# BBillot/SynthSR

Measured on AMD Instinct MI355X. Metric: training volumes/sec (160^3 fp32, 5-level U-Net), higher is better.
Workload: dtype f32; 1 GPU; configs[1]: brain_generator 160^3 batch=1 (training() defaults) + 5-level 3-D U-Net (24..384 features, Cin=2) fwd/bwd + Adam, fp32, random-init; global_batch=1, parallelism=dp1, conv_arithmetic=split

## Files before the change

### synthsr_amd/csrc/conv_split.hip

```cpp
#include "common.h"
#include <algorithm>
#include <type_traits>
#include <utility>

#ifdef SYN_SPLIT_TIMING
static __device__ long long* g_tm = nullptr;
extern "C" int synthsr_split_timing_buffer(long long* p) {
  return hipMemcpyToSymbol(HIP_SYMBOL(g_tm), &p, sizeof(p)) == hipSuccess ? 0 : 1;
}
#define TM(i) do { if (g_tm && (blockIdx.x == 0 || blockIdx.x == 300) && blockIdx.y == 0 && tid == 0 && tix < 120) g_tm[((blockIdx.x ? 1 : 0) * 120 + tix) * 8 + (i)] = clock64(); } while (0)
#define T2(k) do { if (g_tm && threadIdx.x == 0 && ((blockIdx.x == 7 && blockIdx.y == 0) || (blockIdx.x == 20 && blockIdx.y == 1)) && n2 < 400) { g_tm[(blockIdx.y * 400 + n2) * 2] = (k); g_tm[(blockIdx.y * 400 + n2) * 2 + 1] = clock64(); ++n2; } } while (0)
#else
#define TM(i)
#define T2(k)
#endif
#ifdef SYN_SPLIT_TIMING
#define T3(i) do { if (g_tm && lane == 0 && blockIdx.x == 7 && blockIdx.y == 0 && n3 < 48) g_tm[1600 + ((tid >> 6) * 48 + n3) * 2 + (i)] = clock64(); } while (0)
#else
#define T3(i)
#endif


namespace {

// ... 836 lines not shown
    int j = tid + NTHR * i;
    if (j >= NP) j -= NTHR;
    const int v = j >> 1, h = j & 1;
    const int hz = v / (HY * HX), r = v - hz * (HY * HX), hy = r / HX, hx = r - hy * HX;
    prel[i] = ((hz * D1 + hy) * D2 + hx) * Cin * 4 + h * 16;
    plds[i] = v * 16 + h * 8;
    pmask[i] = (1u << hz) | (1u << (6 + hy)) | (1u << (12 + hx));
  }
  const __amdgpu_buffer_rsrc_t rin =
      __builtin_amdgcn_make_buffer_rsrc(const_cast<float*>(a.in), 0, (int)((int64_t)D0 * D1 * D2 * Cin * 4), 0x00020000);
  f32x4 hst[NL], hnx[NL];
  auto halo_issue = [&](int t, int cc) {
    const bool none = t >= walk.end;
    int z0, y0, x0;
    tile_decode(none ? walk.pos : t, tiles0, a.tiles1, a.tiles2, z0, y0, x0);
    uint32_t bad = none ? 0xFFFFFFFFu : 0x80000000u;
    bad |= syn_oob_bits(z0 - 1, HZ, D0) | (syn_oob_bits(y0 - 1, HY, D1) << 6) | (syn_oob_bits(x0 - 1, HX, D2) << 12);
    const int base = ((((z0 - 1) * D1 + (y0 - 1)) * D2 + (x0 - 1)) * Cin + cc * 8) * 4;
#pragma unroll
    for (int i = 0; i < NL; ++i) {
      const uint32_t vo = (pmask[i] & bad) ? OOB : (uint32_t)(prel[i] + base);
      hnx[i] = __builtin_bit_cast(f32x4, __builtin_amdgcn_raw_buffer_load_b128(rin, (int)vo, 0, 0));
    }
  };
  typedef unsigned int u32x2 __attribute__((ext_vector_type(2)));
  uint32_t cp[6];
  auto conv_a = [&](int i) { syn_split3(hst[i][0], hst[i][1], cp[0], cp[1], cp[2]); };
  auto conv_b = [&](int i) { syn_split3(hst[i][2], hst[i][3], cp[3], cp[4], cp[5]); };
  auto conv_c = [&](int i, unsigned char* dst) {
    *reinterpret_cast<u32x2*>(dst + plds[i]) = (u32x2){cp[0], cp[3]};
    *reinterpret_cast<u32x2*>(dst + PLANE + plds[i]) = (u32x2){cp[1], cp[4]};
    *reinterpret_cast<u32x2*>(dst + 2 * PLANE + plds[i]) = (u32x2){cp[2], cp[5]};
  };

  const int piece_stride = nchunks * ncc * NSTEP * MT * 64;
  const __amdgpu_buffer_rsrc_t rw = __builtin_amdgcn_make_buffer_rsrc(
      const_cast<u32x4*>(a.wp), 0, (int)((int64_t)3 * piece_stride * 16), 0x00020000);
  int wsrc[C::NWL];
#pragma unroll
  for (int k = 0; k < C::NWL; ++k) {
    int j = tid + NTHR * k;
    if (j >= C::NWP) j = tid;
    const int q = j / (NSTEP * MT * 64), r = j - q * (NSTEP * MT * 64);
    wsrc[k] = (q * piece_stride + chunk * ncc * NSTEP * MT * 64 + r) * 16;
  }
  u32x4 wst[C::NWL];
  auto w_issue = [&](int cc) {
#pragma unroll
    for (int k = 0; k < C::NWL; ++k) wst[k] = __builtin_amdgcn_raw_buffer_load_b128(rw, wsrc[k] + cc * (NSTEP * MT * 64 * 16), 0, 0);
  };
  auto w_store = [&](unsigned char* dst) {
#pragma unroll
    for (int k = 0; k < C::NWL; ++k) {
      const int j = (tid + NTHR * k) >= C::NWP ? tid : tid + NTHR * k;
      *reinterpret_cast<u32x4*>(dst + j * 16) = wst[k];
    }
  };

  float s1[ST ? MT : 1][4], s2[ST ? MT : 1][4];
#pragma unroll
  for (int mt = 0; mt < (ST ? MT : 1); ++mt)
#pragma unroll
    for (int i = 0; i < 4; ++i) s1[mt][i] = s2[mt][i] = 0.f;

  const int64_t out_bytes = (int64_t)D0 * D1 * D2 * Cout * 4;
  const __amdgpu_buffer_rsrc_t rout = __builtin_amdgcn_make_buffer_rsrc(a.out, 0, (int)out_bytes, 0x00020000);
  const __amdgpu_buffer_rsrc_t radd = __builtin_amdgcn_make_buffer_rsrc(
      const_cast<float*>(a.addend ? a.addend : a.out), 0, (int)out_bytes, 0x00020000);
  const uint32_t ystep = (uint32_t)(D2 * Cout * 4);
  if (tid < MT * 16) {
    const int co = chunk * MT * 16 + tid;
    lbias[tid] = (a.bias && co < Cout) ? a.bias[co] : 0.f;
  }

  f32x4 acc[RW][MT], pend[RW][MT];
  uint32_t prow0 = OOB, pyok = 0;
  f32x4 ev, eb[EPI >= 2 ? NITEM : 1];
  uint32_t eoff;
  auto item_off = [&](int j, uint32_t row0, uint32_t yok) -> uint32_t {
    const int mt = j / RW, y = j % RW;
    const int co = (chunk * MT + mt) * 16 + 4 * g;
    return (((yok >> y) & 1u) && co < Cout) ? row0 + (uint32_t)y * ystep + (uint32_t)(co * 4) : OOB;
  };
  auto addend_issue = [&](uint32_t row0, uint32_t yok) {
    if constexpr (EPI >= 2) {
#pragma unroll
      for (int j = 0; j < NITEM; ++j)
        eb[j] = __builtin_bit_cast(f32x4, __builtin_amdgcn_raw_buffer_load_b128(radd, (int)item_off(j, row0, yok), 0, 0));
    }
  };
  auto epi0 = [&](int j, uint32_t row0, uint32_t yok) { eoff = item_off(j, row0, yok); };
  auto epi1 = [&](int j, const f32x4& src) {
    const f32x4 bj = *reinterpret_cast<const f32x4*>(lbias + (j / RW) * 16 + 4 * g);
    f32x4 v = src;
#pragma unroll
    for (int i = 0; i < 4; ++i) v[i] += bj[i];
    if constexpr (EPI == 2) {
#pragma unroll
      for (int i = 0; i < 4; ++i) v[i] *= act_dy<RELU>(eb[EPI >= 2 ? j : 0][i]);
    }
    if constexpr (EPI == 3 || EPI == 4) {
#pragma unroll
      for (int i = 0; i < 4; ++i) v[i] += eb[EPI >= 2 ? j : 0][i];
    }
    if constexpr (EPI == 1 || EPI == 4) {
#pragma unroll
      for (int i = 0; i < 4; ++i) v[i] = act_f<RELU>(v[i]);
    }
    ev = v;
  };
  auto epi2 = [&](int j) {
    __builtin_amdgcn_raw_buffer_store_b128(__builtin_bit_cast(u32x4, ev), rout, (int)eoff, 0, 0);
    if constexpr (ST) {
      const int mt = j / RW;
      const float w = eoff != OOB ? 1.f : 0.f;
#pragma unroll
      for (int i = 0; i < 4; ++i) {
        const float r = w * ev[i];
        s1[mt][i] += r;
        s2[mt][i] += r * r;
      }
    }
  };
  auto tile_rows = [&](int t, uint32_t& row0, uint32_t& yok) {
    int z0, y0, x0;
    tile_decode(t, tiles0, a.tiles1, a.tiles2, z0, y0, x0);
    const int gz = z0 + zw, gx = x0 + xv, gy = y0 + RW * yh;
    const bool zx_ok = gz < D0 && gx < D2;
    row0 = (uint32_t)((gz * D1 + gy) * D2 + gx) * (uint32_t)(Cout * 4);
    yok = 0;
#pragma unroll
    for (int y = 0; y < RW; ++y) yok |= (zx_ok && (gy + y) < D1) ? (1u << y) : 0u;
  };

  u32x4 wa[2][3][MT], xb[2][3][RW];
  int buf = 0;
  if (walk.pos < walk.end) {
    halo_issue(walk.pos, 0);
    w_issue(0);
#pragma unroll
    for (int i = 0; i < NL; ++i) hst[i] = hnx[i];
#pragma unroll
    for (int i = 0; i < NL; ++i) {
      conv_a(i);
      conv_b(i);
      conv_c(i, lds);
    }
    w_store(wlds);
    const int t1 = ncc > 1 ? walk.pos : walk.pos + walk.stride, c1 = ncc > 1 ? 1 : 0;
    halo_issue(t1, c1);
#pragma unroll
    for (int i = 0; i < NL; ++i) hst[i] = hnx[i];
    const bool last1 = c1 + 1 == ncc;
    halo_issue(last1 ? t1 + walk.stride : t1, last1 ? 0 : c1 + 1);
  }
  auto body = [&](int t, int cc, auto WITH_EPI) {
    constexpr bool WE = decltype(WITH_EPI)::value;
    __syncthreads();
    const bool last_cc = cc + 1 == ncc;
    const int t1 = last_cc ? t + walk.stride : t, c1 = last_cc ? 0 : cc + 1;
    const bool last1 = c1 + 1 == ncc;
    const int t2 = last1 ? t1 + walk.stride : t1, c2 = last1 ? 0 : c1 + 1;
    const bool last2 = c2 + 1 == ncc;
    const int t3 = last2 ? t2 + walk.stride : t2, c3 = last2 ? 0 : c2 + 1;
    w_issue(c1);
    const unsigned char* img = lds + buf * BUF + lbase;
    unsigned char* nimg = lds + (buf ^ 1) * BUF;
    const unsigned char* wl = wlds + (WDB ? buf * C::WBYTES : 0) + lane * 16;
    auto frags = [&](auto SS, auto PP) {
      constexpr int s = decltype(SS)::value, q = decltype(PP)::value;
#pragma unroll
      for (int mt = 0; mt < MT; ++mt)
        wa[s & 1][q][mt] = *reinterpret_cast<const u32x4*>(wl + ((q * NSTEP + s) * MT + mt) * 1024);
#pragma unroll
      for (int y = 0; y < RW; ++y) xb[s & 1][q][y] = *reinterpret_cast<const u32x4*>(img + q * PLANE + koff[s] + y * (HX * 16));
    };
    auto mma = [&](auto SS, auto QA, auto QB) {
      constexpr int s = decltype(SS)::value, qa = decltype(QA)::value, qb = decltype(QB)::value;
#pragma unroll
      for (int y = 0; y < RW; ++y)
#pragma unroll
        for (int mt = 0; mt < MT; ++mt)
          acc[y][mt] = __builtin_amdgcn_mfma_f32_16x16x32_bf16(__builtin_bit_cast(bf16x8, wa[s & 1][qa][mt]),
                                                               __builtin_bit_cast(bf16x8, xb[s & 1][qb][y]), acc[y][mt], 0, 0, 0);
    };
    using I0 = std::integral_constant<int, 0>;
    using I1 = std::integral_constant<int, 1>;
    using I2 = std::integral_constant<int, 2>;
    frags(I0{}, I2{});
    frags(I0{}, I1{});
    frags(I0{}, I0{});
    sfor<0, NSTEP>([&](auto S) {
      constexpr int s = decltype(S)::value;
      constexpr bool last = s + 1 == NSTEP;
      using SN = std::integral_constant<int, last ? 0 : s + 1>;
      constexpr int ci = s - (NSTEP - NL);
      constexpr bool cv = ci >= 0;
      constexpr bool ep = WE && s < NITEM;
      __builtin_amdgcn_sched_barrier(0);
      mma(S, I0{}, I2{});
      __builtin_amdgcn_sched_barrier(0);
      if constexpr (!last) frags(SN{}, I2{});
      if constexpr (ep) epi0(s, prow0, pyok);
      if constexpr (cv) conv_a(ci);
      __builtin_amdgcn_sched_barrier(0);
      mma(S, I0{}, I1{});
      __builtin_amdgcn_sched_barrier(0);
      if constexpr (ep) epi1(s, pend[s % RW][s / RW]);
      __builtin_amdgcn_sched_barrier(0);
      mma(S, I0{}, I0{});
      __builtin_amdgcn_sched_barrier(0);
      if constexpr (!last) frags(SN{}, I1{});
      if constexpr (cv) conv_b(ci);
      __builtin_amdgcn_sched_barrier(0);
      mma(S, I1{}, I0{});
      __builtin_amdgcn_sched_barrier(0);
      if constexpr (ep) epi2(s);
      __builtin_amdgcn_sched_barrier(0);
      mma(S, I1{}, I1{});
      __builtin_amdgcn_sched_barrier(0);
      if constexpr (!last) frags(SN{}, I0{});
      if constexpr (cv) conv_c(ci, nimg);
      __builtin_amdgcn_sched_barrier(0);
      mma(S, I2{}, I0{});
    });
    __builtin_amdgcn_sched_barrier(0);
#pragma unroll
    for (int i = 0; i < NL; ++i) hst[i] = hnx[i];
    halo_issue(t3, c3);
    if constexpr (!WDB) __syncthreads();
    w_store(wlds + (WDB ? (buf ^ 1) * C::WBYTES : 0));
    buf ^= 1;
  };
  auto zero_acc = [&]() {
#pragma unroll
    for (int y = 0; y < RW; ++y)
#pragma unroll
      for (int mt = 0; mt < MT; ++mt) acc[y][mt] = (f32x4){0.f, 0.f, 0.f, 0.f};
  };
#pragma unroll
  for (int y = 0; y < RW; ++y)
#pragma unroll
    for (int mt = 0; mt < MT; ++mt) pend[y][mt] = (f32x4){0.f, 0.f, 0.f, 0.f};
  if (walk.pos < walk.end) {
    for (int t = walk.pos; t < walk.end; t += walk.stride) {
      zero_acc();
      body(t, 0, std::true_type{});
      for (int cc = 1; cc < ncc; ++cc) body(t, cc, std::false_type{});
#pragma unroll
      for (int y = 0; y < RW; ++y)
#pragma unroll
        for (int mt = 0; mt < MT; ++mt) pend[y][mt] = acc[y][mt];
      tile_rows(t, prow0, pyok);
      addend_issue(prow0, pyok);
    }
#pragma unroll
    for (int j = 0; j < NITEM; ++j) {
      epi0(j, prow0, pyok);
      epi1(j, pend[j % RW][j / RW]);
      epi2(j);
    }
  }
  if constexpr (ST) {
    __syncthreads();
    float* red = reinterpret_cast<float*>(lds);
#pragma unroll
    for (int mt = 0; mt < MT; ++mt)
#pragma unroll
      for (int i = 0; i < 4; ++i) {
        float x1 = s1[mt][i], x2 = s2[mt][i];
#pragma unroll
        for (int o = 8; o > 0; o >>= 1) {
          x1 += __shfl_xor(x1, o, 64);
          x2 += __shfl_xor(x2, o, 64);
        }
        if (m == 0) {
          red[(wave * 2 + 0) * (MT * 16) + mt * 16 + 4 * g + i] = x1;
          red[(wave * 2 + 1) * (MT * 16) + mt * 16 + 4 * g + i] = x2;
        }
      }
    __syncthreads();
    float* dst = a.stats_partial + (int64_t)blockIdx.x * (2 * Cout);
    for (int e = tid; e < MT * 16; e += NTHR) {
      const int c = chunk * MT * 16 + e;
      if (c < Cout) {
        float t1 = 0.f, t2 = 0.f;
#pragma unroll
        for (int w = 0; w < 8; ++w) {
          t1 += red[(w * 2 + 0) * (MT * 16) + e];
          t2 += red[(w * 2 + 1) * (MT * 16) + e];
        }
        dst[c] = t1;
        dst[Cout + c] = t2;
      }
    }
  }
}

template <int MT, int NPAR, int NPROD = 6, bool RELU = false>
__global__ __launch_bounds__(512, 1) void conv3d_split_upfwd_kernel(const SplitFwdArgs a) {
  extern __shared__ __attribute__((aligned(16))) unsigned char lds[];
  constexpr int NTHR = 512, WPP = 8 / NPAR, NR = 16 / WPP, NH = NR / 4;
  static_assert(NPAR == 2 || NPAR == 4, "two or four parities per workgroup");
  const int tid = threadIdx.x, lane = tid & 63;
  const int wave = __builtin_amdgcn_readfirstlane(tid >> 6);
  const int m = lane & 15, g = lane >> 4, q = wave % NPAR, part = wave / NPAR;
  const int pg = blockIdx.z;
  const TileWalk walk = tile_walk(a.ntiles);
  const int tiles0 = a.ntiles / (a.tiles1 * a.tiles2);
  const int D0 = a.D0, D1 = a.D1, D2 = a.D2, Cin = a.Cin, Cout = a.Cout, ncc = a.ncc;

  int koff[2];
#pragma unroll
  for (int s = 0; s < 2; ++s) {
    const int t8 = syn_split_tap8(4 * s + g);
    koff[s] = (((t8 >> 2) * HY + ((t8 >> 1) & 1)) * HX + (t8 & 1)) * 16;
  }
  const int xv = syn_split_voxel(m);
  const int par = pg * NPAR + q, pz = (par >> 2) & 1, py = (par >> 1) & 1, px = par & 1;
  const int zw0 = part * NH;
  const int lbase = ((zw0 * HY) * HX + xv) * 16 + ((pz * HY + py) * HX + px) * 16;

  constexpr int NP = HVOX * 2, NL = (NP + NTHR - 1) / NTHR;
  int prel[NL], plds[NL];
  uint32_t pmask[NL];
#pragma unroll
  for (int i = 0; i < NL; ++i) {
    const int j = tid + NTHR * i;
    const int v = j >> 1, h = j & 1;
    const int hz = v / (HY * HX), r = v - hz * (HY * HX), hy = r / HX, hx = r - hy * HX;
    prel[i] = ((hz * D1 + hy) * D2 + hx) * Cin * 4 + h * 16;
    plds[i] = v * 16 + h * 8;
    pmask[i] = j < NP ? ((1u << hz) | (1u << (6 + hy)) | (1u << (12 + hx))) : 0xFFFFFFFFu;
  }
  const __amdgpu_buffer_rsrc_t rin =
      __builtin_amdgcn_make_buffer_rsrc(const_cast<float*>(a.in), 0, (int)((int64_t)D0 * D1 * D2 * Cin * 4), 0x00020000);
  f32x4 stg[NL];
  auto load_halo = [&](int t, int cc) {
    int z0, y0, x0;
    tile_decode(t, tiles0, a.tiles1, a.tiles2, z0, y0, x0);
    uint32_t bad = 0x80000000u;
    bad |= syn_oob_bits(z0 - 1, HZ, D0) | (syn_oob_bits(y0 - 1, HY, D1) << 6) | (syn_oob_bits(x0 - 1, HX, D2) << 12);
    const int base = ((((z0 - 1) * D1 + (y0 - 1)) * D2 + (x0 - 1)) * Cin + cc * 8) * 4;
#pragma unroll
    for (int i = 0; i < NL; ++i) {
      const uint32_t vo = (pmask[i] & bad) ? OOB : (uint32_t)(prel[i] + base);
      stg[i] = __builtin_bit_cast(f32x4, __builtin_amdgcn_raw_buffer_load_b128(rin, (int)vo, 0, 0));
    }
  };
  auto store_halo = [&](int buf) {
    typedef unsigned int u32x2 __attribute__((ext_vector_type(2)));
    unsigned char* dst = lds + buf * BUF;
#pragma unroll
    for (int i = 0; i < NL; ++i) {
      if (i == NL - 1 && tid + NTHR * i >= NP) continue;
      uint32_t p0, p1, p2, q0, q1, q2;
      syn_split3(stg[i][0], stg[i][1], p0, p1, p2);
      syn_split3(stg[i][2], stg[i][3], q0, q1, q2);
      *reinterpret_cast<u32x2*>(dst + plds[i]) = (u32x2){p0, q0};
      *reinterpret_cast<u32x2*>(dst + PLANE + plds[i]) = (u32x2){p1, q1};
      *reinterpret_cast<u32x2*>(dst + 2 * PLANE + plds[i]) = (u32x2){p2, q2};
    }
  };

  const int64_t piece_stride = (int64_t)ncc * 2 * MT * 64, par_stride = 3 * piece_stride;
  const u32x4* __restrict__ wbase = a.wp + (int64_t)par * par_stride + lane;
  u32x4 wa[2][3][MT], xb[3][4];
  auto wload = [&](int cc, int s, int slot) {
#pragma unroll
    for (int pc = 0; pc < 3; ++pc)
#pragma unroll
      for (int mt = 0; mt < MT; ++mt) wa[slot][pc][mt] = wbase[pc * piece_stride + ((cc * 2 + s) * MT + mt) * 64];
  };

  const int64_t out_bytes = (int64_t)8 * D0 * D1 * D2 * Cout * 4;
  const __amdgpu_buffer_rsrc_t rout = __builtin_amdgcn_make_buffer_rsrc(a.out, 0, (int)out_bytes, 0x00020000);
  const __amdgpu_buffer_rsrc_t radd = __builtin_amdgcn_make_buffer_rsrc(
      const_cast<float*>(a.addend ? a.addend : a.out), 0, (int)out_bytes, 0x00020000);

  int buf = 0;
  if (walk.pos < walk.end) {
    load_halo(walk.pos, 0);
    store_halo(0);
    wload(0, 0, 0);
  }
  for (int t = walk.pos; t < walk.end; t += walk.stride) {
    f32x4 acc[NR][MT];
#pragma unroll
    for (int y = 0; y < NR; ++y)
#pragma unroll
      for (int mt = 0; mt < MT; ++mt) acc[y][mt] = (f32x4){0.f, 0.f, 0.f, 0.f};
    for (int cc = 0; cc < ncc; ++cc) {
      __syncthreads();
      const bool more = cc + 1 < ncc || t + walk.stride < walk.end;
      if (cc + 1 < ncc) load_halo(t, cc + 1);
      else if (t + walk.stride < walk.end) load_halo(t + walk.stride, 0);
      const unsigned char* img = lds + buf * BUF + lbase;
      const int cc_next = cc + 1 < ncc ? cc + 1 : 0;
      sfor<0, 2>([&](auto S) {
        constexpr int s = decltype(S)::value, slot = s;
        sfor<0, NH>([&](auto H) {
          constexpr int h = decltype(H)::value;
          __builtin_amdgcn_sched_barrier(0);
#pragma unroll
          for (int pc = 0; pc < 3; ++pc)
#pragma unroll
            for (int y = 0; y < 4; ++y)
              xb[pc][y] = *reinterpret_cast<const u32x4*>(img + pc * PLANE + koff[s] + (h * HY + y) * (HX * 16));
          if constexpr (h == 0) {
            if constexpr (s == 0) wload(cc, 1, 1);
            else wload(cc_next, 0, 0);
          }
          __builtin_amdgcn_sched_barrier(0);
          sfor<0, NPROD>([&](auto CC) {
            constexpr int c = decltype(CC)::value;
            constexpr int qa = split_combo_a(c, NPROD), qb = split_combo_b(c, NPROD);
#pragma unroll
            for (int y = 0; y < 4; ++y)
#pragma unroll
              for (int mt = 0; mt < MT; ++mt)
                acc[4 * h + y][mt] = __builtin_amdgcn_mfma_f32_16x16x32_bf16(
                    __builtin_bit_cast(bf16x8, wa[slot][qa][mt]), __builtin_bit_cast(bf16x8, xb[qb][y]), acc[4 * h + y][mt], 0, 0, 0);
          });
        });
      });
      __builtin_amdgcn_sched_barrier(0);
      if (more) store_halo(buf ^ 1);
      buf ^= 1;
    }
    int z0, y0, x0;
    tile_decode(t, tiles0, a.tiles1, a.tiles2, z0, y0, x0);
    const int gx = x0 + xv;
#pragma unroll
    for (int mt = 0; mt < MT; ++mt) {
      const int co = mt * 16 + 4 * g;
      f32x4 bias = {0.f, 0.f, 0.f, 0.f};
      if (a.bias && co < Cout) bias = *reinterpret_cast<const f32x4*>(a.bias + co);
#pragma unroll
      for (int r = 0; r < NR; ++r) {
        const int gz = z0 + zw0 + (r >> 2), gy = y0 + (r & 3);
        const bool vok = gz < D0 && gx < D2 && gy < D1 && co < Cout;
        const uint32_t off = vok ? (uint32_t)(((2 * gz + pz) * (2 * D1) + (2 * gy + py)) * (2 * D2) + (2 * gx + px)) *
                                       (uint32_t)(Cout * 4) + (uint32_t)(co * 4)
                                 : OOB;
        f32x4 v;
#pragma unroll
        for (int i = 0; i < 4; ++i) v[i] = acc[r][mt][i] + bias[i];
        if (a.addend) {
          const f32x4 b = __builtin_bit_cast(f32x4, __builtin_amdgcn_raw_buffer_load_b128(radd, (int)off, 0, 0));
#pragma unroll
          for (int i = 0; i < 4; ++i) v[i] += b[i];
        }
        if (a.act == 1) {
#pragma unroll
          for (int i = 0; i < 4; ++i) v[i] = act_f<RELU>(v[i]);
        }
        __builtin_amdgcn_raw_buffer_store_b128(__builtin_bit_cast(u32x4, v), rout, (int)off, 0, 0);
      }
    }
  }
}

inline int split_upfwd_grid_x(int ntiles, int ngroups) { return syn_tile_grid_x(256 / ngroups, ntiles); }
inline int split_grid_x(int ntiles, int nchunks) { return syn_tile_grid_x(512 / nchunks, ntiles); }
inline int split_wgrad_grid_x(int ntiles, int gy) {
  int gx = std::max(1, 256 / gy);
  if (gx > ntiles) gx = ntiles;
  return gx;
}

inline int split_tiles1(const int s[3]) { return (s[1] + TY - 1) / TY; }
inline int split_tiles2(const int s[3]) { return (s[2] + TX - 1) / TX; }
inline int split_ntiles(const int s[3]) { return ((s[0] + TZ - 1) / TZ) * split_tiles1(s) * split_tiles2(s); }

inline SplitFwdArgs split_fwd_args(const float* in, const float* wp, const float* bias, const float* addend, float* out,
                                   float* stats_partial, const int s[3], int Cin, int Cout, int act, int stacked) {
  SplitFwdArgs a;
  a.in = in;
  a.wp = reinterpret_cast<const u32x4*>(wp);
  a.bias = bias;
  a.addend = addend;
  a.out = out;
  a.stats_partial = stats_partial;
  a.D0 = s[0]; a.D1 = s[1]; a.D2 = s[2];
  a.Cin = Cin; a.Cout = Cout; a.ncc = Cin / 8;
  a.tiles1 = split_tiles1(s);
  a.tiles2 = split_tiles2(s);
  a.ntiles = split_ntiles(s);
  a.act = act;
  a.stacked = stacked;
  return a;
}

template <class F>
int with_mt(int mt, F&& f) {
  if (mt == 1) return f(std::integral_constant<int, 1>{});
  if (mt == 2) return f(std::integral_constant<int, 2>{});
  return f(std::integral_constant<int, 3>{});
}
inline int split_epi(const SplitFwdArgs& a) {
  if (a.act == 3) return a.addend ? 7 : 5;
  if (a.act == 4) return 6;
  return a.act + ((a.addend && a.act < 2) ? 3 : 0);
}
template <bool ST, class F>
int with_epi(int epi, F&& f) {
  if constexpr (ST) {
    if (epi == 5) return f(std::integral_constant<int, 5>{});
    return epi == 1 ? f(std::integral_constant<int, 1>{}) : f(std::integral_constant<int, 0>{});
  } else {
    switch (epi) {
      case 0: return f(std::integral_constant<int, 0>{});
      case 1: return f(std::integral_constant<int, 1>{});
      case 2: return f(std::integral_constant<int, 2>{});
      case 3: return f(std::integral_constant<int, 3>{});
      case 5: return f(std::integral_constant<int, 5>{});
      case 6: return f(std::integral_constant<int, 6>{});
      case 7: return f(std::integral_constant<int, 7>{});
      default: return f(std::integral_constant<int, 4>{});
    }
  }
}

inline bool relu_args(const SplitFwdArgs& a, SplitFwdArgs& b) {
  b = a;
  if (a.act < 3) return false;
  b.act -= 2;
  return true;
}

template <int MT, int NPAR>
int launch_split_upfwd(const SplitFwdArgs& a0, int nprod, hipStream_t st) {
  constexpr int NG = 8 / NPAR;
  constexpr auto k9r = conv3d_split_upfwd_kernel<MT, NPAR, 9, true>, k9 = conv3d_split_upfwd_kernel<MT, NPAR, 9>;
  constexpr auto k6r = conv3d_split_upfwd_kernel<MT, NPAR, 6, true>, k6 = conv3d_split_upfwd_kernel<MT, NPAR, 6>;
  SplitFwdArgs a;
  const bool relu = relu_args(a0, a);
  const dim3 grid(split_upfwd_grid_x(a.ntiles, NG), 1, NG);
  if (nprod == 9) launch_smem<k9, k9r>(relu, grid, dim3(512), 2 * BUF, st, a);
  else launch_smem<k6, k6r>(relu, grid, dim3(512), 2 * BUF, st, a);
  SYN_CHECK_LAUNCH();
  return SYNTHSR_OK;
}

enum class FwdRoute { generic, fwd2, fwd2_halves, fwd3, refuse };
inline FwdRoute split_fwd_route(int ntiles, int nchunks, int ncc, int mt, int Cout, int stacked, int upm, int nprod) {
  if (stacked) return (upm == 0 && mt == 2 && nprod == 6) ? FwdRoute::fwd2 : FwdRoute::refuse;
  if (upm != 0 || nprod != 6) return FwdRoute::generic;
  const int64_t units = (int64_t)ntiles * nchunks;
  if (!syn_split_replanned(ntiles, (Cout + 15) / 16, mt) && nchunks >= 2 && units >= 512 && units < 1024) return FwdRoute::fwd3;
  const bool halves = (int64_t)split_grid_x(ntiles, nchunks) * nchunks <= 256 && ncc >= 4 && (ncc % 2) == 0;
  return halves ? FwdRoute::fwd2_halves : FwdRoute::fwd2;
}
inline int split_fwd_grid_x(FwdRoute route, int ntiles, int nchunks) {
  return route == FwdRoute::fwd3 ? split_upfwd_grid_x(ntiles, nchunks) : split_grid_x(ntiles, nchunks);
}

template <auto Kern>
int launch_split_fwd_k(const SplitFwdArgs& a, dim3 grid, int threads, size_t smem, hipStream_t st) {
  max_dyn_smem<Kern>(smem);
  hipLaunchKernelGGL(Kern, grid, dim3(threads), smem, st, a);
  SYN_CHECK_LAUNCH();
  return SYNTHSR_OK;
}

template <int MT, bool ST, int UPM>
int launch_split_fwd(const SplitFwdArgs& a0, FwdRoute route, int nchunks, int nprod, hipStream_t st) {
  if (route == FwdRoute::refuse) return SYNTHSR_EINVAL;
  const dim3 grid(split_fwd_grid_x(route, a0.ntiles, nchunks), nchunks);
  if constexpr (UPM == 0) {
    const int epi = split_epi(a0);
    if (a0.stacked) {
      if constexpr (MT == 2)
        return with_epi<ST>(epi, [&](auto E) {
          return launch_split_fwd_k<conv3d_split_fwd2_kernel<2, ST, decltype(E)::value, true>>(a0, grid, 256, 2 * BUF2 + 2 * 16 * 4, st);
        });
      return SYNTHSR_EINVAL;
    }
    if (route == FwdRoute::fwd3)
      return with_epi<ST>(epi, [&](auto E) {
        return launch_split_fwd_k<conv3d_split_fwd3_kernel<MT, ST, decltype(E)::value>>(a0, grid, 512, F3Cfg<MT>::SMEM, st);
      });
    if (route != FwdRoute::generic)
      return with_epi<ST>(epi, [&](auto E) {
        constexpr int EPI = decltype(E)::value;
        if (route == FwdRoute::fwd2_halves)
          return launch_split_fwd_k<conv3d_split_fwd2_kernel<MT, ST, EPI, false, 2>>(a0, grid, 512, 4 * BUF2 + MT * 16 * 4, st);
        return launch_split_fwd_k<conv3d_split_fwd2_kernel<MT, ST, EPI, false>>(a0, grid, 256, 2 * BUF2 + MT * 16 * 4, st);
      });
  }
  constexpr auto k9r = conv3d_split_fwd_kernel<MT, ST, UPM, 9, true>, k9 = conv3d_split_fwd_kernel<MT, ST, UPM, 9>;
  constexpr auto k6r = conv3d_split_fwd_kernel<MT, ST, UPM, 6, true>, k6 = conv3d_split_fwd_kernel<MT, ST, UPM, 6>;
  SplitFwdArgs a;
  const bool relu = relu_args(a0, a);
  if (nprod == 9) launch_smem<k9, k9r>(relu, grid, dim3(256), 2 * BUF, st, a);
  else launch_smem<k6, k6r>(relu, grid, dim3(256), 2 * BUF, st, a);
  SYN_CHECK_LAUNCH();
  return SYNTHSR_OK;
}

typedef short s16x4 __attribute__((ext_vector_type(4)));
typedef __attribute__((address_space(3))) s16x4 lds_s16x4;
__device__ __forceinline__ u32x4 tr_read8(const unsigned char* p_lo, const unsigned char* p_hi) {
  const s16x4 lo = __builtin_amdgcn_ds_read_tr16_b64_v4i16((lds_s16x4*)p_lo);
  const s16x4 hi = __builtin_amdgcn_ds_read_tr16_b64_v4i16((lds_s16x4*)p_hi);
  return __builtin_bit_cast(u32x4, __builtin_shufflevector(lo, hi, 0, 1, 2, 3, 4, 5, 6, 7));
}

struct SplitWgArgs {
  const float* in;
  const float* dout;
  float* dw;
  float* dbias;
  int D0, D1, D2, Cin, Cout, cin_total, ci_off, ncc, nco, tiles1, tiles2, ntiles, ciw;
  int64_t det_stride;
};

template <int COW, int CIW = 8>
struct WgCfg {
  static constexpr int NT = (COW + 15) / 16, DROWB = COW * 2, DPLANE = TZ * TY * TX * DROWB;
  static constexpr int XB = CIW * 2, XPLANE = HVOX * XB;
  static constexpr int NRT = CIW == 24 ? 44 : 14 * (CIW / 8);
  static constexpr int RT = CIW == 24 ? 11 : (COW <= 24 ? 14 : 7);
  static constexpr int BUFB = 3 * XPLANE + 3 * DPLANE + 64;
  static constexpr bool DBUF = 2 * BUFB <= 160 * 1024;
  static constexpr int NBUF = DBUF ? 2 : 1;
};

template <int COW, int NPROD = 6, bool STK = false, int CIW = 8>
__global__ __launch_bounds__(512, 1) void conv3d_split_wgrad_kernel(const SplitWgArgs a) {
  constexpr bool PL = CIW == 24, BAL = CIW == 24;
  constexpr int QP = HVOX * 8;
  static_assert(!STK || (COW == 24 && NPROD == 6), "stacked column tiles: 24 columns, six products");
  static_assert(CIW == 8 || (CIW == 16 && COW == 48) || (CIW == 24 && COW == 24 && STK),
                "16 input channels per workgroup: the 48-column kernel; 24: the stacked 24-column kernel");
  using C = WgCfg<COW, CIW>;
  constexpr int NT = C::NT, DROWB = C::DROWB, DPLANE = C::DPLANE, RT = C::RT, NW = 8, NTHR = 512;
  constexpr int XB = C::XB, WG_XPLANE = C::XPLANE, XQ = CIW / 4;
  constexpr int NXP = HVOX * XQ, NXL = (NXP + NTHR - 1) / NTHR;
  constexpr int DQ = COW / 4, NDP = TZ * TY * TX * DQ, NDL = NDP / NTHR;
  static_assert(NDP % NTHR == 0, "dz pieces divide among the threads");
  extern __shared__ __attribute__((aligned(16))) unsigned char lds[];
  const int tid = threadIdx.x, lane = tid & 63, wave = tid >> 6;
  const int g = lane >> 4, li = lane & 15, lrow = li >> 2, lq = li & 3;
  constexpr int GROUPS = C::NRT / RT, WPG = NW / GROUPS, KPW = 8 / WPG;
  const int rh = CIW == 24 ? __builtin_amdgcn_readfirstlane(wave / WPG) : wave / WPG, wg = wave % WPG;
  const int rt0 = BAL ? rh * (RT - 1) + (rh > 0 ? 1 : 0) : rh * RT;
  const bool slot10 = !BAL || rh == 0 || rh == GROUPS - 1;
  const int cc = blockIdx.y % a.ncc, oc = blockIdx.y / a.ncc;
  const TileWalk walk = tile_walk(a.ntiles);
  const int tiles0 = a.ntiles / (a.tiles1 * a.tiles2);
  const int D0 = a.D0, D1 = a.D1, D2 = a.D2, Cin = a.Cin, Cout = a.Cout;

  int aoff[RT];
#pragma unroll
  for (int q = 0; q < RT; ++q) {
    const int Q = 4 * (rt0 + q) + lq;
    int tap = CIW == 8 ? 2 * (rh * RT + q) + (lq >> 1) : (CIW == 16 ? rh * RT + q : Q / 6);
    if (tap > 26) tap = 26;
    const int tvox = (tap / 9 * HY + (tap / 3) % 3) * HX + tap % 3;
    if constexpr (PL) aoff[q] = tvox * 8 + (Q % 6) * QP;
    else aoff[q] = tvox * XB + (CIW == 8 ? (lq & 1) : (CIW == 16 ? lq : Q % 6)) * 8;
  }
  const int ks0 = wg * KPW, kz = ks0 >> 1, kyb = 2 * (ks0 & 1);
  constexpr int XVB = PL ? 8 : XB;
  auto akoff = [](int kj) { return (uint32_t)(((kj >> 1) * HY * HX + (kj & 1) * 2 * HX) * XVB); };
  auto bkoff = [](int kj) { return (uint32_t)(((kj >> 1) * TY * TX + (kj & 1) * 2 * TX) * DROWB); };
  static_assert(KPW == 1 || KPW == 2 || KPW == 4, "K steps of a wave: whole x-row pairs of consecutive z planes");
  const int vx = 4 * (g & 1) + lrow, vr = g >> 1;
  const uint32_t abase = (uint32_t)((((kz * HY + kyb + vr) * HX) + vx) * XVB);
  const uint32_t bbase = (uint32_t)(3 * WG_XPLANE) + (uint32_t)((((kz * TY + kyb + vr) * TX) + vx) * DROWB + lq * 8);
  constexpr uint32_t ZOFF = (uint32_t)(3 * WG_XPLANE + 3 * DPLANE);
  const uint32_t bvox = bbase - (uint32_t)(lq * 8);
  const uint32_t u3off = bvox + (uint32_t)((lq >> 1) * DPLANE + 32 + (lq & 1) * 8);
  const uint32_t u4off = lq < 2 ? bvox + (uint32_t)(2 * DPLANE + 32 + (lq & 1) * 8) : ZOFF;
  const uint32_t u4hi = lq < 2 ? (uint32_t)(8 * DROWB) : 0u;
  auto u4koff = [&](int kj) { return lq < 2 ? bkoff(kj) : 0u; };
  if constexpr (STK) {
    if (tid < 2 * C::NBUF) *reinterpret_cast<uint64_t*>(lds + (tid >> 1) * C::BUFB + ZOFF + (tid & 1) * 8) = 0ull;
  }

  static_assert(XB == XQ * 8 && DROWB == DQ * 8, "pieces tile the voxel rows");
  constexpr bool XPLN = CIW == 16;
  static_assert(!XPLN || (NXL == HZ && NTHR / XQ >= HY * HX), "one halo plane per staging piece");
  int xrel[XPLN ? 1 : NXL];
  uint32_t xmask[XPLN ? 1 : NXL];
  const int xq = tid & 3, xr = tid >> 2;
  const int xps = D1 * D2 * Cin * 4;
  if constexpr (XPLN) {
    const int hy = xr / HX, hx = xr - hy * HX;
    xrel[0] = (hy * D2 + hx) * Cin * 4 + xq * 16;
    xmask[0] = xr < HY * HX ? ((1u << (6 + hy)) | (1u << (12 + hx))) : 0xFFFFFFFFu;
  } else {
#pragma unroll
    for (int i = 0; i < NXL; ++i) {
      const int j = tid + NTHR * i;
      const int v = j / XQ, h = j % XQ;
      const int hz = v / (HY * HX), r = v - hz * (HY * HX), hy = r / HX, hx = r - hy * HX;
      xrel[i] = ((hz * D1 + hy) * D2 + hx) * Cin * 4 + h * 16;
      xmask[i] = j < NXP ? ((1u << hz) | (1u << (6 + hy)) | (1u << (12 + hx))) : 0xFFFFFFFFu;
    }
  }
  constexpr bool DPLN = XPLN && COW == 48;
  int drel[DPLN ? 1 : NDL];
  uint32_t dmask[DPLN ? 1 : NDL];
  const int dps = 2 * D1 * D2 * Cout * 4;
  if constexpr (DPLN) {
    static_assert(!DPLN || NDL == 6, "two plane pairs x three quad groups");
    const int vz = xr / (TY * TX), vy = (xr / TX) % TY, vxx = xr % TX;
    dmask[0] = (1u << vz) | (1u << (4 + vy)) | (1u << (8 + vxx));
    drel[0] = ((vz * D1 + vy) * D2 + vxx) * Cout * 4 + (oc * COW + xq * 4) * 4;
  } else {
#pragma unroll
    for (int i = 0; i < NDL; ++i) {
      const int j = tid + NTHR * i;
      const int v = j / DQ, c4 = j - v * DQ;
      const int vz = v / (TY * TX), vy = (v / TX) % TY, vxx = v % TX;
      const int co = oc * COW + c4 * 4;
      dmask[i] = co < Cout ? ((1u << vz) | (1u << (4 + vy)) | (1u << (8 + vxx))) : 0xFFFFFFFFu;
      drel[i] = ((vz * D1 + vy) * D2 + vxx) * Cout * 4 + co * 4;
    }
  }
  const __amdgpu_buffer_rsrc_t rin =
      __builtin_amdgcn_make_buffer_rsrc(const_cast<float*>(a.in), 0, (int)((int64_t)D0 * D1 * D2 * Cin * 4), 0x00020000);
  const __amdgpu_buffer_rsrc_t rdo =
      __builtin_amdgcn_make_buffer_rsrc(const_cast<float*>(a.dout), 0, (int)((int64_t)D0 * D1 * D2 * Cout * 4), 0x00020000);
  f32x4 xst[NXL], dst[NDL];
  auto load_tile = [&](int t) {
    int z0, y0, x0;
    tile_decode(t, tiles0, a.tiles1, a.tiles2, z0, y0, x0);
    uint32_t bad = 0x80000000u;
    bad |= syn_oob_bits(z0 - 1, HZ, D0) | (syn_oob_bits(y0 - 1, HY, D1) << 6) | (syn_oob_bits(x0 - 1, HX, D2) << 12);
    const int base = ((((z0 - 1) * D1 + (y0 - 1)) * D2 + (x0 - 1)) * Cin + cc * CIW) * 4;
    int xps_t = xps;
    uint32_t xm_t = xmask[0];
    if constexpr (XPLN) {
      asm volatile("" : "+s"(xps_t));
      asm volatile("" : "+v"(xm_t));
    }
#pragma unroll
// ... 575 lines not shown
```

Before: 53.93 volumes/s.

## Interleave halo LDS store into MFMA loop and cache halo request offsets per tile

In the upsampling split-bf16 forward conv kernel, the LDS store of the prefetched halo moves from after the MFMA loop into the middle of the compute sweep. The weight prefetch is shifted to the same midpoint so LDS writes overlap with matrix work. Halo global offsets are now computed once per tile, and each channel chunk only adds a constant stride, replacing per-thread precomputed arrays to reduce register pressure. An asm barrier on the bias index and restructured weight pointer arithmetic steer codegen. The trade-off is tighter scheduling constraints and possible LDS hazards if the store overlaps reads of the other buffer.

New measurement: 53.68 volumes/s. No clear change (-0.5%).

```diff
diff --git a/synthsr_amd/csrc/conv_split.hip b/synthsr_amd/csrc/conv_split.hip
--- a/synthsr_amd/csrc/conv_split.hip
+++ b/synthsr_amd/csrc/conv_split.hip
@@ -1162,6 +1162,7 @@
   extern __shared__ __attribute__((aligned(16))) unsigned char lds[];
   constexpr int NTHR = 512, WPP = 8 / NPAR, NR = 16 / WPP, NH = NR / 4;
   static_assert(NPAR == 2 || NPAR == 4, "two or four parities per workgroup");
+  constexpr int SS = NH == 1 ? 1 : 0;
   const int tid = threadIdx.x, lane = tid & 63;
   const int wave = __builtin_amdgcn_readfirstlane(tid >> 6);
   const int m = lane & 15, g = lane >> 4, q = wave % NPAR, part = wave / NPAR;
@@ -1182,55 +1183,57 @@
   const int lbase = ((zw0 * HY) * HX + xv) * 16 + ((pz * HY + py) * HX + px) * 16;
 
   constexpr int NP = HVOX * 2, NL = (NP + NTHR - 1) / NTHR;
-  int prel[NL], plds[NL];
-  uint32_t pmask[NL];
-#pragma unroll
-  for (int i = 0; i < NL; ++i) {
-    const int j = tid + NTHR * i;
-    const int v = j >> 1, h = j & 1;
-    const int hz = v / (HY * HX), r = v - hz * (HY * HX), hy = r / HX, hx = r - hy * HX;
-    prel[i] = ((hz * D1 + hy) * D2 + hx) * Cin * 4 + h * 16;
-    plds[i] = v * 16 + h * 8;
-    pmask[i] = j < NP ? ((1u << hz) | (1u << (6 + hy)) | (1u << (12 + hx))) : 0xFFFFFFFFu;
-  }
+  const int plds0 = (tid >> 1) * 16 + (tid & 1) * 8;
   const __amdgpu_buffer_rsrc_t rin =
       __builtin_amdgcn_make_buffer_rsrc(const_cast<float*>(a.in), 0, (int)((int64_t)D0 * D1 * D2 * Cin * 4), 0x00020000);
   f32x4 stg[NL];
-  auto load_halo = [&](int t, int cc) {
+  uint32_t vo[NL];
+  auto halo_requests = [&](int t) {
     int z0, y0, x0;
     tile_decode(t, tiles0, a.tiles1, a.tiles2, z0, y0, x0);
     uint32_t bad = 0x80000000u;
     bad |= syn_oob_bits(z0 - 1, HZ, D0) | (syn_oob_bits(y0 - 1, HY, D1) << 6) | (syn_oob_bits(x0 - 1, HX, D2) << 12);
-    const int base = ((((z0 - 1) * D1 + (y0 - 1)) * D2 + (x0 - 1)) * Cin + cc * 8) * 4;
+    const int base = ((((z0 - 1) * D1 + (y0 - 1)) * D2 + (x0 - 1)) * Cin) * 4;
 #pragma unroll
     for (int i = 0; i < NL; ++i) {
-      const uint32_t vo = (pmask[i] & bad) ? OOB : (uint32_t)(prel[i] + base);
-      stg[i] = __builtin_bit_cast(f32x4, __builtin_amdgcn_raw_buffer_load_b128(rin, (int)vo, 0, 0));
-    }
+      const int j = tid + NTHR * i;
+      const int v = j >> 1, h = j & 1;
+      const int hz = v / (HY * HX), r = v - hz * (HY * HX), hy = r / HX, hx = r - hy * HX;
+      const uint32_t mask = j < NP ? ((1u << hz) | (1u << (6 + hy)) | (1u << (12 + hx))) : 0xFFFFFFFFu;
+      vo[i] = (mask & bad) ? OOB : (uint32_t)(((hz * D1 + hy) * D2 + hx) * Cin * 4 + h * 16 + base);
+    }
+  };
+  auto load_halo = [&](int cc) {
+#pragma unroll
+    for (int i = 0; i < NL; ++i)
+      stg[i] = __builtin_bit_cast(f32x4, __builtin_amdgcn_raw_buffer_load_b128(rin, (int)(vo[i] + (uint32_t)(cc * 32)), 0, 0));
   };
   auto store_halo = [&](int buf) {
     typedef unsigned int u32x2 __attribute__((ext_vector_type(2)));
-    unsigned char* dst = lds + buf * BUF;
+    unsigned char* dst = lds + buf * BUF + plds0;
 #pragma unroll
     for (int i = 0; i < NL; ++i) {
       if (i == NL - 1 && tid + NTHR * i >= NP) continue;
       uint32_t p0, p1, p2, q0, q1, q2;
       syn_split3(stg[i][0], stg[i][1], p0, p1, p2);
       syn_split3(stg[i][2], stg[i][3], q0, q1, q2);
-      *reinterpret_cast<u32x2*>(dst + plds[i]) = (u32x2){p0, q0};
-      *reinterpret_cast<u32x2*>(dst + PLANE + plds[i]) = (u32x2){p1, q1};
-      *reinterpret_cast<u32x2*>(dst + 2 * PLANE + plds[i]) = (u32x2){p2, q2};
+      *reinterpret_cast<u32x2*>(dst + i * (8 * NTHR)) = (u32x2){p0, q0};
+      *reinterpret_cast<u32x2*>(dst + PLANE + i * (8 * NTHR)) = (u32x2){p1, q1};
+      *reinterpret_cast<u32x2*>(dst + 2 * PLANE + i * (8 * NTHR)) = (u32x2){p2, q2};
     }
   };
 
   const int64_t piece_stride = (int64_t)ncc * 2 * MT * 64, par_stride = 3 * piece_stride;
-  const u32x4* __restrict__ wbase = a.wp + (int64_t)par * par_stride + lane;
+  const u32x4* __restrict__ wpar = a.wp + (int64_t)par * par_stride;
+  const uint32_t wlane = (uint32_t)lane;
   u32x4 wa[2][3][MT], xb[3][4];
   auto wload = [&](int cc, int s, int slot) {
 #pragma unroll
-    for (int pc = 0; pc < 3; ++pc)
-#pragma unroll
-      for (int mt = 0; mt < MT; ++mt) wa[slot][pc][mt] = wbase[pc * piece_stride + ((cc * 2 + s) * MT + mt) * 64];
+    for (int pc = 0; pc < 3; ++pc) {
+      const u32x4* __restrict__ wp = wpar + (pc * piece_stride + (cc * 2 + s) * MT * 64);
+#pragma unroll
+      for (int mt = 0; mt < MT; ++mt) wa[slot][pc][mt] = wp[mt * 64 + wlane];
+    }
   };
 
   const int64_t out_bytes = (int64_t)8 * D0 * D1 * D2 * Cout * 4;
@@ -1240,7 +1243,8 @@
 
   int buf = 0;
   if (walk.pos < walk.end) {
-    load_halo(walk.pos, 0);
+    halo_requests(walk.pos);
+    load_halo(0);
     store_halo(0);
     wload(0, 0, 0);
   }
@@ -1253,8 +1257,11 @@
     for (int cc = 0; cc < ncc; ++cc) {
       __syncthreads();
       const bool more = cc + 1 < ncc || t + walk.stride < walk.end;
-      if (cc + 1 < ncc) load_halo(t, cc + 1);
-      else if (t + walk.stride < walk.end) load_halo(t + walk.stride, 0);
+      if (cc + 1 < ncc) load_halo(cc + 1);
+      else if (t + walk.stride < walk.end) {
+        halo_requests(t + walk.stride);
+        load_halo(0);
+      }
       const unsigned char* img = lds + buf * BUF + lbase;
       const int cc_next = cc + 1 < ncc ? cc + 1 : 0;
       sfor<0, 2>([&](auto S) {
@@ -1262,12 +1269,16 @@
         sfor<0, NH>([&](auto H) {
           constexpr int h = decltype(H)::value;
           __builtin_amdgcn_sched_barrier(0);
+          if constexpr (s == SS && h == NH / 2) {
+            if (more) store_halo(buf ^ 1);
+            __builtin_amdgcn_sched_barrier(0);
+          }
 #pragma unroll
           for (int pc = 0; pc < 3; ++pc)
 #pragma unroll
             for (int y = 0; y < 4; ++y)
               xb[pc][y] = *reinterpret_cast<const u32x4*>(img + pc * PLANE + koff[s] + (h * HY + y) * (HX * 16));
-          if constexpr (h == 0) {
+          if constexpr (h == NH / 2) {
             if constexpr (s == 0) wload(cc, 1, 1);
             else wload(cc_next, 0, 0);
           }
@@ -1285,7 +1296,6 @@
         });
       });
       __builtin_amdgcn_sched_barrier(0);
-      if (more) store_halo(buf ^ 1);
       buf ^= 1;
     }
     int z0, y0, x0;
@@ -1295,7 +1305,9 @@
     for (int mt = 0; mt < MT; ++mt) {
       const int co = mt * 16 + 4 * g;
       f32x4 bias = {0.f, 0.f, 0.f, 0.f};
-      if (a.bias && co < Cout) bias = *reinterpret_cast<const f32x4*>(a.bias + co);
+      int cb = co;
+      asm volatile("" : "+v"(cb));
+      if (a.bias && co < Cout) bias = *reinterpret_cast<const f32x4*>(a.bias + cb);
 #pragma unroll
       for (int r = 0; r < NR; ++r) {
         const int gz = z0 + zw0 + (r >> 2), gy = y0 + (r & 3);
```
